# matthiasverstraete/3d_recognizer

Measured on AMD Instinct MI355X. Metric: training clouds/sec, N=40960 pts, bs=8, at 1/2/4/8 GPUs; mIoU parity, higher is better.
Workload: dtype f32 storage/accumulate, bf16x3 MFMA in the wide GEMMs

## Files before the change

### 3d_recognizer_amd/csrc/csr.hip

```cpp
#include "rl_common.h"

namespace {

constexpr int CSR_MAX_TASKS = 8;

struct CsrTask {
    const int32_t* idx;
    int n_src, k, n_dst;
    int32_t* offsets;
    int32_t* entries;
    int32_t* tmp;
    int32_t* cursor;
    int32_t* long_list;
    int32_t* long_count;
    int long_cap;
    int cap;
    int nbuckets;
    int ntiles;
    int32_t* bsize;
    int32_t* bstart;
};
struct CsrMulti {
    CsrTask t[CSR_MAX_TASKS];
    int ntasks;
    int B;
    int xcd;
};

__device__ __forceinline__ void csr_deal(const CsrMulti& m, int& b, int& bx) {
    if (m.xcd) {
        const int lin = (int)blockIdx.x + (int)gridDim.x * b;
        b = lin % m.B;
        bx = lin / m.B;
    }
}

__global__ __launch_bounds__(256) void csr_zero_kernel(const CsrMulti m) {
    const CsrTask& T = m.t[blockIdx.y];
    const long total = (long)m.B * T.n_dst;
    for (long e = (long)blockIdx.x * 256 + threadIdx.x; e < total; e += (long)gridDim.x * 256) T.cursor[e] = 0;
    if (blockIdx.x == 0 && threadIdx.x == 0) T.long_count[0] = 0;
}

__global__ __launch_bounds__(256) void csr_count_kernel(const CsrMulti m) {
    const CsrTask& T = m.t[blockIdx.y];
    const unsigned per = (unsigned)T.n_src * (unsigned)T.k;
    const long total = (long)m.B * per;
    for (long e = (long)blockIdx.x * 256 + threadIdx.x; e < total; e += (long)gridDim.x * 256) {
        const unsigned b = (unsigned)e / per;
        const int j = T.idx[e];
        if ((unsigned)j < (unsigned)T.n_dst) atomicAdd(&T.cursor[(long)b * T.n_dst + j], 1);
    }
}

__global__ __launch_bounds__(1024) void csr_scan_kernel(const CsrMulti m) {
    __shared__ int part[1024];
    const int task = blockIdx.x / m.B, b = blockIdx.x % m.B, t = threadIdx.x;
    const CsrTask& T = m.t[task];
    int* cu = T.cursor + (long)b * T.n_dst;
    int* off = T.offsets + (long)b * (T.n_dst + 1);
    const int chunk = (T.n_dst + 1023) / 1024;
    const int lo = min(T.n_dst, t * chunk), hi = min(T.n_dst, lo + chunk);
    int s = 0;
    for (int i = lo; i < hi; ++i) s += cu[i];
    part[t] = s;
    __syncthreads();
    for (int o = 1; o < 1024; o <<= 1) {
        const int v = (t >= o) ? part[t - o] : 0;
// ... 5 lines not shown
    for (int i = lo; i < hi; ++i) {
        const int c = cu[i];
        off[i] = run;
        cu[i] = run;
        run += c;
    }
    if (t == 1023) off[T.n_dst] = part[1023];
}

__global__ __launch_bounds__(256) void csr_fill_kernel(const CsrMulti m) {
    const CsrTask& T = m.t[blockIdx.y];
    const unsigned per = (unsigned)T.n_src * (unsigned)T.k;
    const long total = (long)m.B * per;
    for (long e = (long)blockIdx.x * 256 + threadIdx.x; e < total; e += (long)gridDim.x * 256) {
        const unsigned b = (unsigned)e / per;
        const int j = T.idx[e];
        if ((unsigned)j >= (unsigned)T.n_dst) continue;
        const int pos = atomicAdd(&T.cursor[(long)b * T.n_dst + j], 1);
        T.tmp[(long)b * per + pos] = (int)((unsigned)e - b * per);
    }
}

constexpr int CSR_TILE = 4096;
constexpr int CSR_BUCKET = 256;
constexpr int CSR_MAX_BUCKETS = 1024;

__global__ __launch_bounds__(256) void csr2_zero_kernel(const CsrMulti m) {
    const CsrTask& T = m.t[blockIdx.y];
    const long total = (long)m.B * T.nbuckets;
    for (long e = (long)blockIdx.x * 256 + threadIdx.x; e < total; e += (long)gridDim.x * 256) T.bsize[e] = 0;
    if (blockIdx.x == 0 && threadIdx.x == 0) T.long_count[0] = 0;
}

__global__ __launch_bounds__(256) void csr2_hist_kernel(const CsrMulti m) {
    __shared__ int hist[CSR_MAX_BUCKETS];
    const int task = blockIdx.y / m.B;
    int b = blockIdx.y % m.B, bx = blockIdx.x;
    csr_deal(m, b, bx);
    const CsrTask& T = m.t[task];
    if (bx >= T.ntiles) return;
    const int per = T.n_src * T.k;
    for (int i = threadIdx.x; i < T.nbuckets; i += 256) hist[i] = 0;
    __syncthreads();
    const int32_t* idx = T.idx + (long)b * per;
    const int e0 = bx * CSR_TILE;
#pragma unroll 4
    for (int i = 0; i < CSR_TILE / 256; ++i) {
        const int e = e0 + i * 256 + threadIdx.x;
        if (e < per) {
            const int j = idx[e];
            if ((unsigned)j < (unsigned)T.n_dst) atomicAdd(&hist[j >> 8], 1);
        }
    }
    __syncthreads();
    for (int i = threadIdx.x; i < T.nbuckets; i += 256)
        if (hist[i] > 0) atomicAdd(&T.bsize[(long)b * T.nbuckets + i], hist[i]);
}

__global__ __launch_bounds__(1024) void csr2_scan_kernel(const CsrMulti m) {
    __shared__ int part[1024];
    const int task = blockIdx.x / m.B, b = blockIdx.x % m.B, t = threadIdx.x;
    const CsrTask& T = m.t[task];
    int* bs = T.bsize + (long)b * T.nbuckets;
    const int v = t < T.nbuckets ? bs[t] : 0;
    part[t] = v;
    __syncthreads();
    for (int o = 1; o < 1024; o <<= 1) {
        const int u = (t >= o) ? part[t - o] : 0;
        __syncthreads();
        part[t] += u;
        __syncthreads();
    }
    int* st = T.bstart + (long)b * (T.nbuckets + 1);
    if (t < T.nbuckets) {
        st[t] = part[t] - v;
        bs[t] = 0;
    }
    if (t == T.nbuckets - 1) st[T.nbuckets] = part[t];
}

__global__ __launch_bounds__(256) void csr2_scatter_kernel(const CsrMulti m) {
    __shared__ int hist[CSR_MAX_BUCKETS];
    const int task = blockIdx.y / m.B;
    int b = blockIdx.y % m.B, bx = blockIdx.x;
    csr_deal(m, b, bx);
    const CsrTask& T = m.t[task];
    if (bx >= T.ntiles) return;
    const int per = T.n_src * T.k;
    for (int i = threadIdx.x; i < T.nbuckets; i += 256) hist[i] = 0;
    __syncthreads();
    const int32_t* idx = T.idx + (long)b * per;
    const int e0 = bx * CSR_TILE;
    int jv[CSR_TILE / 256], rk[CSR_TILE / 256];
#pragma unroll
    for (int i = 0; i < CSR_TILE / 256; ++i) {
        const int e = e0 + i * 256 + threadIdx.x;
        jv[i] = -1;
        if (e < per) {
            const int j = idx[e];
            if ((unsigned)j < (unsigned)T.n_dst) {
                jv[i] = j;
                rk[i] = atomicAdd(&hist[j >> 8], 1);
            }
        }
    }
    __syncthreads();
    for (int i = threadIdx.x; i < T.nbuckets; i += 256) {
        const int c = hist[i];
        hist[i] = c > 0 ? atomicAdd(&T.bsize[(long)b * T.nbuckets + i], c) : 0;
    }
    __syncthreads();
    const int* st = T.bstart + (long)b * (T.nbuckets + 1);
    int32_t* mid = T.tmp + (long)b * per;
#pragma unroll
    for (int i = 0; i < CSR_TILE / 256; ++i) {
        if (jv[i] >= 0) {
            const int h = jv[i] >> 8;
            mid[st[h] + hist[h] + rk[i]] = ((jv[i] & 255) << 24) | (e0 + i * 256 + threadIdx.x);
        }
    }
}

template <int CAP>
__global__ __launch_bounds__(256) void csr2_bucket_kernel(const CsrMulti m) {
    __shared__ int cnt[CSR_BUCKET], start[CSR_BUCKET], cur[CSR_BUCKET];
    __shared__ int seg[CSR_BUCKET][CAP + 1];
    const int task = blockIdx.y / m.B;
    int b = blockIdx.y % m.B, bx = blockIdx.x;
    csr_deal(m, b, bx);
    const CsrTask& T = m.t[task];
    if (T.cap != CAP || bx >= T.nbuckets) return;
    const int per = T.n_src * T.k, h = bx, t = threadIdx.x;
    const int* st = T.bstart + (long)b * (T.nbuckets + 1);
    const int s0 = st[h], mcount = st[h + 1] - s0;
    const int32_t* mid = T.tmp + (long)b * per + s0;
    int32_t* ent = T.entries + (long)b * per + s0;
    cnt[t] = 0;
    cur[t] = 0;
    __syncthreads();
    for (int e = t; e < mcount; e += 256) atomicAdd(&cnt[(unsigned)mid[e] >> 24], 1);
    __syncthreads();
    const int c = cnt[t];
    start[t] = c;
    __syncthreads();
    for (int o = 1; o < 256; o <<= 1) {
        const int u = (t >= o) ? start[t - o] : 0;
        __syncthreads();
        start[t] += u;
        __syncthreads();
    }
    const int my_start = start[t] - c;
    __syncthreads();
    start[t] = my_start;
    const int j = h * CSR_BUCKET + t;
    int* off = T.offsets + (long)b * (T.n_dst + 1);
    if (j < T.n_dst) off[j] = s0 + my_start;
    if (j == T.n_dst - 1) off[T.n_dst] = st[T.nbuckets];
    __syncthreads();
    for (int e = t; e < mcount; e += 256) {
        const int p = mid[e];
        const int lo = (unsigned)p >> 24, r = p & 0xffffff;
        const int pos = atomicAdd(&cur[lo], 1);
        if (cnt[lo] <= CAP) seg[lo][pos] = r;
        else ent[start[lo] + pos] = r;
// ... 230 lines not shown
    p.long_list = o;  o += up256((size_t)p.long_cap * 4);
    p.long_count = o; o += 256;
    p.bsize = o;      o += up256((size_t)B * p.nbuckets * 4);
    p.bstart = o;     o += up256((size_t)B * (p.nbuckets + 1) * 4);
    p.bytes = o;
    return p;
}
inline bool all_two_level(const rl_csr_task* tasks, int ntasks) {
    for (int i = 0; i < ntasks; ++i)
        if (!two_level_ok(tasks[i])) return false;
    return true;
}

}

extern "C" int64_t rl_csr_workspace_bytes(const rl_csr_task* tasks, int ntasks, int B) {
    if (!tasks || ntasks <= 0 || B <= 0) return 0;
    int64_t total = 0;
    for (int i = 0; i < ntasks; ++i) {
        if (tasks[i].n_src <= 0 || tasks[i].k <= 0 || tasks[i].n_dst <= 0) return 0;
        total += (int64_t)make_plan(B, tasks[i], all_two_level(tasks, ntasks)).bytes;
    }
    return total;
}

extern "C" int rl_csr_build(const rl_csr_task* tasks, int ntasks, int B, void* workspace, int64_t workspace_bytes,
                            void* stream) {
    RL_REQUIRE(tasks && ntasks > 0 && ntasks <= CSR_MAX_TASKS && B > 0 && (long)B * ntasks <= 65535, RL_ERR_ARGS,
               "rl_csr_build: 1..%d tasks expected", CSR_MAX_TASKS);
    RL_REQUIRE(workspace && ((uintptr_t)workspace & 255) == 0, RL_ERR_ARGS, "rl_csr_build: workspace must be 256-byte aligned");
    CsrMulti m;
    m.ntasks = ntasks;
    m.B = B;
    m.xcd = (B > 1 && 8 % B == 0) ? 1 : 0;
    char* ws = (char*)workspace;
    int64_t used = 0;
    long max_ent = 1, max_dst = 1;
    int max_tiles = 1, max_buckets = 1;
    bool need[3] = {false, false, false};
    for (int i = 0; i < ntasks; ++i)
        RL_REQUIRE(tasks[i].idx && tasks[i].offsets && tasks[i].entries && tasks[i].n_src > 0 && tasks[i].k > 0 && tasks[i].n_dst > 0,
                   RL_ERR_ARGS, "rl_csr_build: bad task %d", i);
    const bool two = all_two_level(tasks, ntasks);
    for (int i = 0; i < ntasks; ++i) {
        const rl_csr_task& t = tasks[i];
        RL_REQUIRE((int64_t)B * t.n_src * t.k < (1l << 31) && (int64_t)B * t.n_dst < (1l << 31), RL_ERR_ARGS,
                   "rl_csr_build: task %d is too large", i);
        const Plan p = make_plan(B, t, two);
        RL_REQUIRE(used + (int64_t)p.bytes <= workspace_bytes, RL_ERR_ARGS, "rl_csr_build: workspace too small");
        CsrTask& T = m.t[i];
        T.idx = t.idx; T.n_src = t.n_src; T.k = t.k; T.n_dst = t.n_dst; T.offsets = t.offsets; T.entries = t.entries;
        T.tmp = (int32_t*)(ws + used + p.tmp);
        T.cursor = (int32_t*)(ws + used + p.cursor);
        T.long_list = (int32_t*)(ws + used + p.long_list);
        T.long_count = (int32_t*)(ws + used + p.long_count);
        T.bsize = (int32_t*)(ws + used + p.bsize);
        T.bstart = (int32_t*)(ws + used + p.bstart);
        T.long_cap = p.long_cap; T.cap = p.cap; T.nbuckets = p.nbuckets; T.ntiles = p.ntiles;
        need[p.cap == 32 ? 0 : (p.cap == 64 || p.cap == 56) ? 1 : 2] = true;
        used += (int64_t)p.bytes;
        max_ent = max_ent > (long)B * t.n_src * t.k ? max_ent : (long)B * t.n_src * t.k;
        max_dst = max_dst > (long)B * t.n_dst ? max_dst : (long)B * t.n_dst;
        max_tiles = max_tiles > p.ntiles ? max_tiles : p.ntiles;
        max_buckets = max_buckets > p.nbuckets ? max_buckets : p.nbuckets;
    }
    hipStream_t st = (hipStream_t)stream;
    auto gridx = [](long work, int per) { long g = (work + per - 1) / per; return (unsigned)(g < 1 ? 1 : (g > 4096 ? 4096 : g)); };
    if (two) {
        hipLaunchKernelGGL(csr2_zero_kernel, dim3(gridx((long)B * max_buckets, 256), ntasks), dim3(256), 0, st, m);
        hipLaunchKernelGGL(csr2_hist_kernel, dim3(max_tiles, ntasks * B), dim3(256), 0, st, m);
        hipLaunchKernelGGL(csr2_scan_kernel, dim3(ntasks * B), dim3(1024), 0, st, m);
        hipLaunchKernelGGL(csr2_scatter_kernel, dim3(max_tiles, ntasks * B), dim3(256), 0, st, m);
        if (need[0]) hipLaunchKernelGGL(csr2_bucket_kernel<32>, dim3(max_buckets, ntasks * B), dim3(256), 0, st, m);
        if (need[1]) hipLaunchKernelGGL(csr2_bucket_kernel<56>, dim3(max_buckets, ntasks * B), dim3(256), 0, st, m);
        hipLaunchKernelGGL(csr2_sort_long_kernel, dim3(128, ntasks), dim3(256), 0, st, m);
        rl_note_kernel("csr2_bucket_kernel");
        RL_LAUNCH_CHECK("rl_csr_build");
        return RL_OK;
    }
    hipLaunchKernelGGL(csr_zero_kernel, dim3(gridx(max_dst, 256), ntasks), dim3(256), 0, st, m);
    hipLaunchKernelGGL(csr_count_kernel, dim3(gridx(max_ent, 256), ntasks), dim3(256), 0, st, m);
    hipLaunchKernelGGL(csr_scan_kernel, dim3(ntasks * B), dim3(1024), 0, st, m);
    hipLaunchKernelGGL(csr_fill_kernel, dim3(gridx(max_ent, 256), ntasks), dim3(256), 0, st, m);
    if (need[0]) hipLaunchKernelGGL((csr_sort_kernel<32, 256>), dim3(gridx(max_dst, 256), ntasks), dim3(256), 0, st, m);
    if (need[1]) hipLaunchKernelGGL((csr_sort_kernel<64, 128>), dim3(gridx(max_dst, 128), ntasks), dim3(128), 0, st, m);
    if (need[2]) hipLaunchKernelGGL((csr_sort_kernel<128, 64>), dim3(gridx(max_dst, 64), ntasks), dim3(64), 0, st, m);
    hipLaunchKernelGGL(csr_sort_long_kernel, dim3(128, ntasks), dim3(256), 0, st, m);
    rl_note_kernel("csr_sort_kernel");
    RL_LAUNCH_CHECK("rl_csr_build");
    return RL_OK;
}

extern "C" int rl_segment_sum_rows(const rl_segsum_desc* d, void* stream) {
    RL_REQUIRE(d && d->src && d->dst && d->offsets && d->entries && d->B > 0 && d->n_dst > 0 && d->C > 0 && d->entries_per_cloud >= 0,
               RL_ERR_ARGS, "rl_segment_sum_rows: bad descriptor");
    RL_REQUIRE(d->lds >= d->C && d->ldd >= d->C && d->dst_bstride >= d->n_dst && d->src_bstride > 0, RL_ERR_ARGS,
               "rl_segment_sum_rows: bad strides");
    RL_REQUIRE((int64_t)d->B * d->n_dst < (1l << 31), RL_ERR_ARGS, "rl_segment_sum_rows: too many rows");
    SegParams p;
    p.src = d->src; p.lds = d->lds; p.src_bstride = d->src_bstride; p.dst = d->dst; p.ldd = d->ldd;
    p.dst_bstride = d->dst_bstride; p.offsets = d->offsets; p.entries = d->entries; p.n_dst = d->n_dst; p.C = d->C;
    p.per = d->entries_per_cloud; p.total = (long)d->B * d->n_dst; p.accumulate = d->accumulate;
    p.xcd_chunk = 0;
    hipStream_t st = (hipStream_t)stream;
    const bool vec = (d->C % 4 == 0) && (d->lds % 4 == 0) && (d->ldd % 4 == 0) && ((uintptr_t)d->dst & 15) == 0 &&
                     ((uintptr_t)d->src & (d->src_bf16 ? 7 : 15)) == 0;
    RL_REQUIRE(!d->src_bf16 || vec, RL_ERR_UNSUPPORTED, "rl_segment_sum_rows: bf16 source rows need C, lds, ldd multiples of 4 and aligned tensors");
// ... 33 lines not shown
```

### 3d_recognizer_amd/csrc/knn_grid.hip

```cpp
#include "rl_common.h"
#include <stdlib.h>

namespace {

constexpr int KNN_SB = 3;


struct GridGeom {
    float lo[3];
    float inv[3];
    float h[3];
    int n[3];
    int ncell;
    float slack;
};

__device__ __forceinline__ unsigned enc(float f) {
    const unsigned u = __float_as_uint(f);
    return (u & 0x80000000u) ? ~u : (u | 0x80000000u);
}
__device__ __forceinline__ float dec(unsigned u) {
    return __uint_as_float((u & 0x80000000u) ? (u & 0x7fffffffu) : ~u);
}

constexpr int KNN_MAX_TASKS = 8;

struct KTask {
    const float* S;
    long s_bs;
    const float* Q;
    long q_bs;
    int Ns, Nq, k, self_mode;
    int32_t* idx32;
    int64_t* idx64;
    float* d2;
    GridGeom* geom;
    unsigned* bbox;
    int* count;
    int* start;
    int* cursor;
    float4* sorted;
    int cstride, maxcells;
    float per_cell;
    int lanes;
};

struct KMulti {
    int ntasks, B;
    int xcd;
    KTask t[KNN_MAX_TASKS];
};

__device__ __forceinline__ void knn_deal(const KMulti& m, int& b, int& bx) {
    if (m.xcd) {
        const int lin = (int)blockIdx.x + (int)gridDim.x * b;
        b = lin % m.B;
        bx = lin / m.B;
    }
}

__device__ __forceinline__ int kmax_of(int k) { return k == 1 ? 1 : k <= 4 ? 4 : k <= 8 ? 8 : k <= 16 ? 16 : k <= 32 ? 32 : 64; }

__global__ __launch_bounds__(256) void grid_init_kernel(const KMulti m) {
    const int task = blockIdx.y / m.B, b = blockIdx.y % m.B;
    const KTask& T = m.t[task];
    const int i = blockIdx.x * 256 + threadIdx.x;
    if (i < 6) T.bbox[b * 6 + i] = (i < 3) ? 0xffffffffu : 0u;
    int* cnt = T.count + (size_t)b * T.cstride;
    for (int e = i; e < T.cstride; e += gridDim.x * 256) cnt[e] = 0;
}

__global__ __launch_bounds__(256) void grid_bbox_kernel(const KMulti m) {
    const int task = blockIdx.y / m.B, b = blockIdx.y % m.B;
    const KTask& T = m.t[task];
    if (blockIdx.x * 256 >= T.Ns) return;
    const float* Sb = T.S + (size_t)b * T.s_bs * 3;
    float mn[3] = {INFINITY, INFINITY, INFINITY}, mx[3] = {-INFINITY, -INFINITY, -INFINITY};
    for (int j = blockIdx.x * 256 + threadIdx.x; j < T.Ns; j += gridDim.x * 256) {
#pragma unroll
        for (int a = 0; a < 3; ++a) {
            const float v = Sb[(size_t)j * 3 + a];
            mn[a] = fminf(mn[a], v);
            mx[a] = fmaxf(mx[a], v);
        }
    }
#pragma unroll
    for (int a = 0; a < 3; ++a) {
#pragma unroll
        for (int o = 32; o > 0; o >>= 1) {
            mn[a] = fminf(mn[a], __shfl_xor(mn[a], o, 64));
            mx[a] = fmaxf(mx[a], __shfl_xor(mx[a], o, 64));
        }
// ... 44 lines not shown
        g.n[a] = n;
        total *= n;
    }
    while (total > T.maxcells) {
        int a = 0;
        if (g.n[1] > g.n[a]) a = 1;
        if (g.n[2] > g.n[a]) a = 2;
        g.n[a] = (g.n[a] + 1) / 2;
        total = (long)g.n[0] * g.n[1] * g.n[2];
    }
    for (int a = 0; a < 3; ++a) {
        g.h[a] = (ext[a] > 0.f) ? ext[a] / (float)g.n[a] : 1.f;
        g.inv[a] = 1.f / g.h[a];
    }
    g.ncell = (int)total;
    g.slack = 1e-5f * extent + 1e-30f;
    T.geom[b] = g;
}

__device__ __forceinline__ void cell_coords(const GridGeom& g, float x, float y, float z, int c[3]) {
    const float p[3] = {x, y, z};
#pragma unroll
    for (int a = 0; a < 3; ++a) {
        int ci = (int)floorf((p[a] - g.lo[a]) * g.inv[a]);
        ci = ci < 0 ? 0 : ci;
        ci = ci >= g.n[a] ? g.n[a] - 1 : ci;
        c[a] = ci;
    }
}
__device__ __forceinline__ int cell_id(const GridGeom& g, const int c[3]) {
    return (c[2] * g.n[1] + c[1]) * g.n[0] + c[0];
}

__global__ __launch_bounds__(256) void grid_count_kernel(const KMulti m) {
    const int task = blockIdx.y / m.B, b = blockIdx.y % m.B;
    const KTask& T = m.t[task];
    const int j = blockIdx.x * 256 + threadIdx.x;
    if (j >= T.Ns) return;
    const GridGeom g = T.geom[b];
    const float* p = T.S + ((size_t)b * T.s_bs + j) * 3;
    int c[3];
    cell_coords(g, p[0], p[1], p[2], c);
    atomicAdd(&T.count[(size_t)b * T.cstride + cell_id(g, c)], 1);
}

__global__ __launch_bounds__(1024) void grid_scan_kernel(const KMulti m) {
    __shared__ int part[1024];
    const int task = blockIdx.x / m.B, b = blockIdx.x % m.B, t = threadIdx.x;
    const KTask& T = m.t[task];
    const int ncell = T.geom[b].ncell;
    const int* cnt = T.count + (size_t)b * T.cstride;
    int* st = T.start + (size_t)b * T.cstride;
    int* cu = T.cursor + (size_t)b * T.cstride;
    const int chunk = (ncell + 1023) / 1024;
    const int lo = t * chunk, hi = min(ncell, lo + chunk);
    int s = 0;
    for (int i = lo; i < hi; ++i) s += cnt[i];
    part[t] = s;
    __syncthreads();
    for (int o = 1; o < 1024; o <<= 1) {
        const int v = (t >= o) ? part[t - o] : 0;
        __syncthreads();
        part[t] += v;
        __syncthreads();
    }
    int run = part[t] - s;
    for (int i = lo; i < hi; ++i) {
        st[i] = run;
        cu[i] = run;
        run += cnt[i];
    }
    if (t == 1023) st[ncell] = part[1023];
}

__global__ __launch_bounds__(256) void grid_scatter_kernel(const KMulti m) {
    const int task = blockIdx.y / m.B, b = blockIdx.y % m.B;
    const KTask& T = m.t[task];
    const int j = blockIdx.x * 256 + threadIdx.x;
    if (j >= T.Ns) return;
    const GridGeom g = T.geom[b];
    const float* p = T.S + ((size_t)b * T.s_bs + j) * 3;
    int c[3];
    cell_coords(g, p[0], p[1], p[2], c);
    const int pos = atomicAdd(&T.cursor[(size_t)b * T.cstride + cell_id(g, c)], 1);
    T.sorted[(size_t)b * T.Ns + pos] = make_float4(p[0], p[1], p[2], __int_as_float(j));
}

constexpr unsigned long long KEY_EMPTY = 0x7FF0000000000000ull;
template <int KMAX>
__device__ __forceinline__ void insert_key(unsigned long long key, unsigned long long (&best)[KMAX]) {
    double kd = __builtin_bit_cast(double, key);
#pragma unroll
    for (int s = 0; s < KMAX; ++s) {
        const double bs = __builtin_bit_cast(double, best[s]);
        double lo, hi;
        asm("v_min_f64 %0, %1, %2" : "=v"(lo) : "v"(kd), "v"(bs));
        asm("v_max_f64 %0, %1, %2" : "=v"(hi) : "v"(kd), "v"(bs));
        best[s] = __builtin_bit_cast(unsigned long long, lo);
        kd = hi;
    }
}

template <int KMAX, int SB>
__device__ __forceinline__ void take_batch(const float4 (&cand)[SB], unsigned valid, float qx, float qy, float qz,
                                           unsigned long long (&best)[KMAX]) {
    unsigned long long key[SB];
    unsigned pass = 0;
#pragma unroll
    for (int i = 0; i < SB; ++i) {
        const float4 c = cand[i];
        const float dx = __fsub_rn(qx, c.x), dy = __fsub_rn(qy, c.y), dz = __fsub_rn(qz, c.z);
        const float d = __fadd_rn(__fadd_rn(__fmul_rn(dx, dx), __fmul_rn(dy, dy)), __fmul_rn(dz, dz));
        key[i] = ((unsigned long long)__float_as_uint(d) << 32) | (unsigned)__float_as_int(c.w);
        if (((valid >> i) & 1u) && key[i] < best[KMAX - 1]) pass |= 1u << i;
    }
    while (pass) {
        const int i = __ffs(pass) - 1;
        pass &= pass - 1;
        unsigned long long kk = key[0];
#pragma unroll
        for (int j = 1; j < SB; ++j)
            if (j == i) kk = key[j];
        insert_key<KMAX>(kk, best);
    }
}

template <int KMAX>
__device__ __forceinline__ void scan_range(const float4* __restrict__ pts, int begin, int end, float qx, float qy,
                                           float qz, unsigned long long (&best)[KMAX]) {
    constexpr int SB = KNN_SB;
    for (int t = begin; t < end; t += SB) {
        float4 cand[SB];
        unsigned valid = 0;
#pragma unroll
        for (int i = 0; i < SB; ++i) {
            cand[i] = pts[min(t + i, end - 1)];
            if (t + i < end) valid |= 1u << i;
        }
        take_batch<KMAX, SB>(cand, valid, qx, qy, qz, best);
    }
}

__device__ __forceinline__ int centre_out(int t) { return (t & 1) ? -((t + 1) >> 1) : (t >> 1); }

__device__ __forceinline__ float axis_gap(const GridGeom& g, int a, int ci, float q) {
    const float lo = g.lo[a] + (float)ci * g.h[a];
    const float hi = lo + g.h[a];
    float gap = fmaxf(lo - q, q - hi);
    gap -= g.slack;
    return gap > 0.f ? gap : 0.f;
}

template <int KMAX>
__device__ __forceinline__ void query_one_lane(const KTask& T, int b, int bx) {
    const int k = T.k, Nq = T.Nq, Ns = T.Ns;
    const int t = bx * 256 + threadIdx.x;
    if (t >= Nq) return;
    const int self_mode = T.self_mode;
    const float* Q = T.Q;
    const long q_bs = T.q_bs;
    int32_t* idx32 = T.idx32;
    int64_t* idx64 = T.idx64;
    float* d2out = T.d2;
    const GridGeom g = T.geom[b];
    const float4* pts = T.sorted + (size_t)b * Ns;
    const int* st = T.start + (size_t)b * T.cstride;
    float qx, qy, qz;
    int qi;
    if (self_mode) {
        const float4 me = pts[t];
        qx = me.x; qy = me.y; qz = me.z;
        qi = __float_as_int(me.w);
    } else {
        const float* p = Q + ((size_t)b * q_bs + t) * 3;
        qx = p[0]; qy = p[1]; qz = p[2];
        qi = t;
    }
    int c[3];
    cell_coords(g, qx, qy, qz, c);
    unsigned long long best[KMAX];
#pragma unroll
    for (int s = 0; s < KMAX; ++s) best[s] = KEY_EMPTY;

    const float q3[3] = {qx, qy, qz};
    for (int r = 0;; ++r) {
        const int z0 = max(c[2] - r, 0), z1 = min(c[2] + r, g.n[2] - 1);
        const int y0 = max(c[1] - r, 0), y1 = min(c[1] + r, g.n[1] - 1);
        const int x0 = max(c[0] - r, 0), x1 = min(c[0] + r, g.n[0] - 1);
        for (int tz = 0; tz <= 2 * r; ++tz) {
            const int z = c[2] + centre_out(tz);
            if (z < z0 || z > z1) continue;
            const bool zedge = (z == c[2] - r) || (z == c[2] + r);
            const float dz = axis_gap(g, 2, z, qz);
            for (int ty = 0; ty <= 2 * r; ++ty) {
                const int y = c[1] + centre_out(ty);
                if (y < y0 || y > y1) continue;
                const bool full_row = zedge || y == c[1] - r || y == c[1] + r;
                const float dy = axis_gap(g, 1, y, qy);
                const float dyz = dy * dy + dz * dz;
                const int row = (z * g.n[1] + y) * g.n[0];
                unsigned long long kth = best[KMAX - 1];
                if (k != KMAX) {
#pragma unroll
                    for (int s = 0; s < KMAX; ++s)
                        if (s == k - 1) kth = best[s];
                }
                const bool have = kth != KEY_EMPTY;
                const float lim = have ? __uint_as_float((unsigned)(kth >> 32)) * 1.00001f + 1e-30f : INFINITY;
                if (dyz > lim) continue;
                if (full_row) {
                    int xa = x0, xb = x1;
                    while (xa <= xb) {
                        const float gx = axis_gap(g, 0, xa, qx);
                        if (gx * gx + dyz > lim) ++xa; else break;
                    }
                    while (xb >= xa) {
                        const float gx = axis_gap(g, 0, xb, qx);
                        if (gx * gx + dyz > lim) --xb; else break;
                    }
                    if (xa <= xb) scan_range<KMAX>(pts, st[row + xa], st[row + xb + 1], qx, qy, qz, best);
                } else {
#pragma unroll
                    for (int e = 0; e < 2; ++e) {
                        const int x = e == 0 ? c[0] - r : c[0] + r;
                        if (x < x0 || x > x1 || (e == 1 && r == 0)) continue;
                        const float dxg = axis_gap(g, 0, x, qx);
                        if (dxg * dxg + dyz > lim) continue;
                        scan_range<KMAX>(pts, st[row + x], st[row + x + 1], qx, qy, qz, best);
                    }
                }
            }
        }
        const bool covers = (c[0] - r <= 0) && (c[0] + r >= g.n[0] - 1) && (c[1] - r <= 0) && (c[1] + r >= g.n[1] - 1) &&
                            (c[2] - r <= 0) && (c[2] + r >= g.n[2] - 1);
        if (covers) break;
        unsigned long long kth = best[KMAX - 1];
#pragma unroll
        for (int s = 0; s < KMAX; ++s)
            if (s == k - 1) kth = best[s];
        if (kth != KEY_EMPTY) {
            float bound = INFINITY;
#pragma unroll
            for (int a = 0; a < 3; ++a) {
                if (c[a] - r > 0) bound = fminf(bound, q3[a] - (g.lo[a] + (float)(c[a] - r) * g.h[a]));
                if (c[a] + r < g.n[a] - 1) bound = fminf(bound, (g.lo[a] + (float)(c[a] + r + 1) * g.h[a]) - q3[a]);
            }
            bound -= g.slack;
            const float kd = __uint_as_float((unsigned)(kth >> 32));
            if (bound > 0.f && kd < bound * bound * 0.999999f) break;
        }
    }
    const size_t o = ((size_t)b * Nq + qi) * k;
#pragma unroll
    for (int s = 0; s < KMAX; ++s) {
        if (s < k) {
            const bool empty = best[s] == KEY_EMPTY;
            const unsigned id = empty ? 0xffffffffu : (unsigned)(best[s] & 0xffffffffull);
            if (idx32) idx32[o + s] = (int32_t)id;
            if (idx64) idx64[o + s] = (int64_t)id;
            d2out[o + s] = __uint_as_float(empty ? 0xffffffffu : (unsigned)(best[s] >> 32));
        }
    }
}

template <int LANES>
__device__ __forceinline__ unsigned long long group_min(unsigned long long v) {
#pragma unroll
// ... 134 lines not shown
        }
    }
#pragma unroll
    for (int s = 0; s < KMAX; ++s) lists[qslot][sub][s] = best[s];
    __syncthreads();
    if (active) {
        const size_t o = ((size_t)b * Nq + qi) * k;
#pragma unroll
        for (int s = 0; s < KMAX; ++s) {
            const unsigned long long key = best[s];
            if (key == KEY_EMPTY) continue;
            int rank = s;
#pragma unroll
            for (int j = 1; j < LANES; ++j) {
                const unsigned long long* L = lists[qslot][(sub + j) % LANES];
                int lo = 0;
#pragma unroll
                for (int w = KMAX / 2; w >= 1; w >>= 1)
                    if (L[lo + w - 1] < key) lo += w;
                if (lo < KMAX && L[lo] < key) ++lo;
                rank += lo;
            }
            if (rank < k) {
                const unsigned id = (unsigned)(key & 0xffffffffull);
                if (T.idx32) T.idx32[o + rank] = (int32_t)id;
                if (T.idx64) T.idx64[o + rank] = (int64_t)id;
                T.d2[o + rank] = __uint_as_float((unsigned)(key >> 32));
            }
        }
    }
}

template <int KMAX>
__global__ __launch_bounds__(256, KMAX <= 16 ? 4 : 1) void grid_query_kernel(const KMulti m) {
    __shared__ unsigned long long lds[KMAX <= 16 ? 256 * KMAX : 1];
    const int task = blockIdx.y / m.B;
    int b = blockIdx.y % m.B, bx = blockIdx.x;
    knn_deal(m, b, bx);
    const KTask& T = m.t[task];
    if (kmax_of(T.k) != KMAX) return;
    if constexpr (KMAX <= 16) {
        if (T.lanes == 4) { query_n_lanes<KMAX, 4>(T, b, bx, lds); return; }
        if (T.lanes == 2) { query_n_lanes<KMAX, 2>(T, b, bx, lds); return; }
    }
    query_one_lane<KMAX>(T, b, bx);
}

struct Plan {
    int maxcells, cstride;
    float per_cell;
    size_t off_geom, off_bbox, off_count, off_start, off_cursor, off_sorted, bytes;
};

Plan make_plan(int B, int Ns, int k) {
    Plan p;
    constexpr float occ = 0.5f;
    p.per_cell = fmaxf(2.f, occ * (float)k);
    const long want = (long)((double)Ns / p.per_cell) + 1;
    p.maxcells = (int)(4 * want + 64);
    p.cstride = p.maxcells + 1;
    size_t o = 0;
    auto take = [&](size_t n) { size_t at = o; o += (n + 255) & ~(size_t)255; return at; };
    p.off_geom = take(sizeof(GridGeom) * B);
    p.off_bbox = take(sizeof(unsigned) * 6 * B);
    p.off_count = take(sizeof(int) * (size_t)p.cstride * B);
    p.off_start = take(sizeof(int) * (size_t)p.cstride * B);
    p.off_cursor = take(sizeof(int) * (size_t)p.cstride * B);
    p.off_sorted = take(sizeof(float4) * (size_t)Ns * B);
    p.bytes = o;
    return p;
}

void bind(KTask* t, const Plan& p, char* w) {
    t->geom = (GridGeom*)(w + p.off_geom);
    t->bbox = (unsigned*)(w + p.off_bbox);
    t->count = (int*)(w + p.off_count);
    t->start = (int*)(w + p.off_start);
    t->cursor = (int*)(w + p.off_cursor);
    t->sorted = (float4*)(w + p.off_sorted);
    t->cstride = p.cstride;
    t->maxcells = p.maxcells;
    t->per_cell = p.per_cell;
}

inline int lanes_for(long queries, int k) {
    if (k > 16) return 1;
    return queries >= 16384 ? 1 : 4;
}

int run_multi(const KMulti& m_in, hipStream_t st) {
    KMulti m = m_in;
    m.xcd = (m.B > 1 && 8 % m.B == 0) ? 1 : 0;
    for (int i = 0; i < m.ntasks; ++i) m.t[i].lanes = lanes_for((long)m.B * m.t[i].Nq, m.t[i].k);
    int maxNs = 1, maxNq = 1, maxc = 1;
    bool need[6] = {false, false, false, false, false, false};
    for (int i = 0; i < m.ntasks; ++i) {
        maxNs = max(maxNs, m.t[i].Ns);
        maxNq = max(maxNq, m.t[i].Nq);
        maxc = max(maxc, m.t[i].cstride);
        const int k = m.t[i].k;
        need[k == 1 ? 0 : k <= 4 ? 1 : k <= 8 ? 2 : k <= 16 ? 3 : k <= 32 ? 4 : 5] = true;
    }
    const int clouds = m.ntasks * m.B;
    int gi = rl_cdiv(maxc, 256);
    if (gi > 64) gi = 64;
    hipLaunchKernelGGL(grid_init_kernel, dim3(gi, clouds), dim3(256), 0, st, m);
    int gb = rl_cdiv(maxNs, 2048);
    if (gb > 16) gb = 16;
    hipLaunchKernelGGL(grid_bbox_kernel, dim3(gb, clouds), dim3(256), 0, st, m);
    hipLaunchKernelGGL(grid_geom_kernel, dim3(rl_cdiv(clouds, 64)), dim3(64), 0, st, m);
    hipLaunchKernelGGL(grid_count_kernel, dim3(rl_cdiv(maxNs, 256), clouds), dim3(256), 0, st, m);
    hipLaunchKernelGGL(grid_scan_kernel, dim3(clouds), dim3(1024), 0, st, m);
    hipLaunchKernelGGL(grid_scatter_kernel, dim3(rl_cdiv(maxNs, 256), clouds), dim3(256), 0, st, m);
    int gxq = 1;
    for (int i = 0; i < m.ntasks; ++i) gxq = max(gxq, rl_cdiv((long)m.t[i].Nq * m.t[i].lanes, 256));
    dim3 grid(gxq, clouds);
    if (need[0]) hipLaunchKernelGGL((grid_query_kernel<1>), grid, dim3(256), 0, st, m);
    if (need[1]) hipLaunchKernelGGL((grid_query_kernel<4>), grid, dim3(256), 0, st, m);
    if (need[2]) hipLaunchKernelGGL((grid_query_kernel<8>), grid, dim3(256), 0, st, m);
    if (need[3]) hipLaunchKernelGGL((grid_query_kernel<16>), grid, dim3(256), 0, st, m);
    if (need[4]) hipLaunchKernelGGL((grid_query_kernel<32>), grid, dim3(256), 0, st, m);
    if (need[5]) hipLaunchKernelGGL((grid_query_kernel<64>), grid, dim3(256), 0, st, m);
    rl_note_kernel("grid_query_kernel");
    RL_LAUNCH_CHECK("rl_knn(grid)");
    return RL_OK;
}

}

int64_t rl_knn_grid_workspace_bytes(int B, int Ns, int k) { return (int64_t)make_plan(B, Ns, k).bytes; }

int rl_knn_grid_run(const float* S, long s_bs, const float* Q, long q_bs, int B, int Ns, int Nq, int k, int32_t* i32,
                    int64_t* i64, float* d2, void* workspace, int64_t workspace_bytes, hipStream_t st) {
    const Plan p = make_plan(B, Ns, k);
    RL_REQUIRE(workspace && workspace_bytes >= (int64_t)p.bytes, RL_ERR_ARGS, "rl_knn: workspace too small (%ld < %ld bytes)",
               (long)workspace_bytes, (long)p.bytes);
    RL_REQUIRE(((uintptr_t)workspace & 255) == 0, RL_ERR_ARGS, "rl_knn: workspace must be 256-byte aligned");
    KMulti m;
    m.ntasks = 1;
    m.B = B;
    KTask& t = m.t[0];
    t.S = S; t.s_bs = s_bs; t.Q = Q; t.q_bs = q_bs; t.Ns = Ns; t.Nq = Nq; t.k = k;
    t.self_mode = (S == Q && s_bs == q_bs && Ns == Nq) ? 1 : 0;
    t.idx32 = i32; t.idx64 = i64; t.d2 = d2;
    bind(&t, p, (char*)workspace);
    return run_multi(m, st);
}

extern "C" int64_t rl_knn_multi_workspace_bytes(const rl_knn_task* tasks, int ntasks, int B) {
    if (!tasks || ntasks <= 0 || B <= 0) return 0;
    int64_t total = 0;
    for (int i = 0; i < ntasks; ++i) total += (int64_t)make_plan(B, tasks[i].Ns, tasks[i].k).bytes;
    return total;
}

// ... 28 lines not shown
```

### 3d_recognizer_amd/csrc/rl_common.h

```cpp
#pragma once
#include <hip/hip_runtime.h>
#include <stdarg.h>
#include <stdint.h>
#include <stdio.h>

#include "../../include/rl_randlanet.h"

void rl_set_error(const char* fmt, ...);
void rl_note_kernel(const char* name);

#define RL_REQUIRE(cond, code, ...)      \
    do {                                 \
        if (!(cond)) {                   \
            rl_set_error(__VA_ARGS__);   \
            return (code);               \
        }                                \
    } while (0)

#define RL_LAUNCH_CHECK(name)                                                        \
    do {                                                                             \
        hipError_t e_ = hipGetLastError();                                           \
        if (e_ != hipSuccess) {                                                      \
            rl_set_error("%s: launch failed: %s", name, hipGetErrorString(e_));      \
            return RL_ERR_LAUNCH;                                                    \
        }                                                                            \
    } while (0)

void rl_count_launch();
#undef hipLaunchKernelGGL
#define hipLaunchKernelGGL(kernelName, numBlocks, numThreads, memPerBlock, streamId, ...)                         \
    do {                                                                                                         \
        rl_count_launch();                                                                                       \
        kernelName<<<(numBlocks), (numThreads), (memPerBlock), (streamId)>>>(__VA_ARGS__);                       \
    } while (0)

int rl_wide_terms();

static inline int rl_cdiv(long a, long b) { return (int)((a + b - 1) / b); }

#include <stdlib.h>
static inline bool rl_float_atomics_allowed() {
    const char* e = getenv("RL_ALLOW_FLOAT_ATOMICS");
    return e && e[0] == '1';
}

static inline int rl_row_blocks_host(long rows, int rows_per_tile) {
    long tiles = (rows + rows_per_tile - 1) / rows_per_tile;
    if (tiles < 1) tiles = 1;
    return (int)(tiles < RL_MAX_SLOTS ? tiles : RL_MAX_SLOTS);
}

#define RL_ACT_NONE 0
#define RL_ACT_RELU 1
#define RL_ACT_LRELU 2

__device__ __forceinline__ float rl_act(float z, int act, float slope) {
    if (act == RL_ACT_RELU) return z > 0.f ? z : 0.f;
    if (act == RL_ACT_LRELU) return z > 0.f ? z : z * slope;
    return z;
}
__device__ __forceinline__ float rl_act_grad(float z, int act, float slope) {
    if (act == RL_ACT_RELU) return z > 0.f ? 1.f : 0.f;
    if (act == RL_ACT_LRELU) return z > 0.f ? 1.f : slope;
    return 1.f;
}

struct RlLazy {
    const float* scale;
    const float* shift;
    int act;
    float slope;
};
__device__ __forceinline__ float rl_lazy(const RlLazy& t, float raw, int c) {
    if (t.scale == nullptr) return raw;
    return rl_act(raw * t.scale[c] + t.shift[c], t.act, t.slope);
}

typedef __bf16 rl_bf16x4 __attribute__((ext_vector_type(4)));
template <bool BF>
__device__ __forceinline__ float rl_ldx(const float* p, long i) {
    if constexpr (BF) return (float)reinterpret_cast<const __bf16*>(p)[i];
    else return p[i];
// ... 60 lines not shown
```

Baseline: 1269.

## Pack multi-task launches into dense dealt grids and defer KNN k=16 inserts via LDS queue

Adds an RlDeal helper that turns per-task block counts into one dense 1D grid, sorted by size and optionally XCD-interleaved, so CSR and KNN kernels no longer launch max_tiles×tasks grids with idle early-exit blocks. The bucket kernels are launched only over tasks with a matching cap. For k=16, the one-lane KNN query now stages candidate keys in a per-thread LDS queue and merges them in wave-uniform batches, reducing divergent insertion-sort work. The two-lane query path is removed, and the queue adds LDS traffic and extra code paths.

Result: no change. 1276 (median of 6 runs) (+0.5%).

```diff
diff --git a/3d_recognizer_amd/csrc/csr.hip b/3d_recognizer_amd/csrc/csr.hip
--- a/3d_recognizer_amd/csrc/csr.hip
+++ b/3d_recognizer_amd/csrc/csr.hip
@@ -3,6 +3,7 @@
 namespace {
 
 constexpr int CSR_MAX_TASKS = 8;
+static_assert(CSR_MAX_TASKS <= RL_DEAL_MAX, "one RlDeal slot per task");
 
 struct CsrTask {
     const int32_t* idx;
@@ -24,16 +25,8 @@
     CsrTask t[CSR_MAX_TASKS];
     int ntasks;
     int B;
-    int xcd;
 };
 
-__device__ __forceinline__ void csr_deal(const CsrMulti& m, int& b, int& bx) {
-    if (m.xcd) {
-        const int lin = (int)blockIdx.x + (int)gridDim.x * b;
-        b = lin % m.B;
-        bx = lin / m.B;
-    }
-}
 
 __global__ __launch_bounds__(256) void csr_zero_kernel(const CsrMulti m) {
     const CsrTask& T = m.t[blockIdx.y];
@@ -105,13 +98,11 @@
     if (blockIdx.x == 0 && threadIdx.x == 0) T.long_count[0] = 0;
 }
 
-__global__ __launch_bounds__(256) void csr2_hist_kernel(const CsrMulti m) {
+__global__ __launch_bounds__(256) void csr2_hist_kernel(const CsrMulti m, const RlDeal deal) {
     __shared__ int hist[CSR_MAX_BUCKETS];
-    const int task = blockIdx.y / m.B;
-    int b = blockIdx.y % m.B, bx = blockIdx.x;
-    csr_deal(m, b, bx);
+    int task, b, bx;
+    if (!rl_deal_find(deal, task, b, bx)) return;
     const CsrTask& T = m.t[task];
-    if (bx >= T.ntiles) return;
     const int per = T.n_src * T.k;
     for (int i = threadIdx.x; i < T.nbuckets; i += 256) hist[i] = 0;
     __syncthreads();
@@ -152,13 +143,11 @@
     if (t == T.nbuckets - 1) st[T.nbuckets] = part[t];
 }
 
-__global__ __launch_bounds__(256) void csr2_scatter_kernel(const CsrMulti m) {
+__global__ __launch_bounds__(256) void csr2_scatter_kernel(const CsrMulti m, const RlDeal deal) {
     __shared__ int hist[CSR_MAX_BUCKETS];
-    const int task = blockIdx.y / m.B;
-    int b = blockIdx.y % m.B, bx = blockIdx.x;
-    csr_deal(m, b, bx);
+    int task, b, bx;
+    if (!rl_deal_find(deal, task, b, bx)) return;
     const CsrTask& T = m.t[task];
-    if (bx >= T.ntiles) return;
     const int per = T.n_src * T.k;
     for (int i = threadIdx.x; i < T.nbuckets; i += 256) hist[i] = 0;
     __syncthreads();
@@ -195,14 +184,13 @@
 }
 
 template <int CAP>
-__global__ __launch_bounds__(256) void csr2_bucket_kernel(const CsrMulti m) {
+__global__ __launch_bounds__(256) void csr2_bucket_kernel(const CsrMulti m, const RlDeal deal) {
     __shared__ int cnt[CSR_BUCKET], start[CSR_BUCKET], cur[CSR_BUCKET];
     __shared__ int seg[CSR_BUCKET][CAP + 1];
-    const int task = blockIdx.y / m.B;
-    int b = blockIdx.y % m.B, bx = blockIdx.x;
-    csr_deal(m, b, bx);
+    int task, b, bx;
+    if (!rl_deal_find(deal, task, b, bx)) return;
     const CsrTask& T = m.t[task];
-    if (T.cap != CAP || bx >= T.nbuckets) return;
+    if (bx >= T.nbuckets) return;
     const int per = T.n_src * T.k, h = bx, t = threadIdx.x;
     const int* st = T.bstart + (long)b * (T.nbuckets + 1);
     const int s0 = st[h], mcount = st[h + 1] - s0;
@@ -499,11 +487,12 @@
     CsrMulti m;
     m.ntasks = ntasks;
     m.B = B;
-    m.xcd = (B > 1 && 8 % B == 0) ? 1 : 0;
+    const bool xcd = B > 1 && 8 % B == 0;
     char* ws = (char*)workspace;
     int64_t used = 0;
     long max_ent = 1, max_dst = 1;
-    int max_tiles = 1, max_buckets = 1;
+    int max_buckets = 1;
+    int tiles[CSR_MAX_TASKS], buckets[2][CSR_MAX_TASKS];
     bool need[3] = {false, false, false};
     for (int i = 0; i < ntasks; ++i)
         RL_REQUIRE(tasks[i].idx && tasks[i].offsets && tasks[i].entries && tasks[i].n_src > 0 && tasks[i].k > 0 && tasks[i].n_dst > 0,
@@ -528,18 +517,26 @@
         used += (int64_t)p.bytes;
         max_ent = max_ent > (long)B * t.n_src * t.k ? max_ent : (long)B * t.n_src * t.k;
         max_dst = max_dst > (long)B * t.n_dst ? max_dst : (long)B * t.n_dst;
-        max_tiles = max_tiles > p.ntiles ? max_tiles : p.ntiles;
+        tiles[i] = p.ntiles;
+        buckets[0][i] = p.cap == 32 ? 1 : 0;
+        buckets[1][i] = p.cap == 32 ? 0 : 1;
         max_buckets = max_buckets > p.nbuckets ? max_buckets : p.nbuckets;
     }
     hipStream_t st = (hipStream_t)stream;
     auto gridx = [](long work, int per) { long g = (work + per - 1) / per; return (unsigned)(g < 1 ? 1 : (g > 4096 ? 4096 : g)); };
     if (two) {
         hipLaunchKernelGGL(csr2_zero_kernel, dim3(gridx((long)B * max_buckets, 256), ntasks), dim3(256), 0, st, m);
-        hipLaunchKernelGGL(csr2_hist_kernel, dim3(max_tiles, ntasks * B), dim3(256), 0, st, m);
+        const RlDeal dt = rl_deal_make(tiles, ntasks, B, xcd);
+        for (int i = 0; i < ntasks; ++i) {
+            buckets[0][i] *= max_buckets;
+            buckets[1][i] *= max_buckets;
+        }
+        const RlDeal db32 = rl_deal_make(buckets[0], ntasks, B, xcd), db56 = rl_deal_make(buckets[1], ntasks, B, xcd);
+        hipLaunchKernelGGL(csr2_hist_kernel, rl_deal_grid(dt), dim3(256), 0, st, m, dt);
         hipLaunchKernelGGL(csr2_scan_kernel, dim3(ntasks * B), dim3(1024), 0, st, m);
-        hipLaunchKernelGGL(csr2_scatter_kernel, dim3(max_tiles, ntasks * B), dim3(256), 0, st, m);
-        if (need[0]) hipLaunchKernelGGL(csr2_bucket_kernel<32>, dim3(max_buckets, ntasks * B), dim3(256), 0, st, m);
-        if (need[1]) hipLaunchKernelGGL(csr2_bucket_kernel<56>, dim3(max_buckets, ntasks * B), dim3(256), 0, st, m);
+        hipLaunchKernelGGL(csr2_scatter_kernel, rl_deal_grid(dt), dim3(256), 0, st, m, dt);
+        if (need[0]) hipLaunchKernelGGL(csr2_bucket_kernel<32>, rl_deal_grid(db32), dim3(256), 0, st, m, db32);
+        if (need[1]) hipLaunchKernelGGL(csr2_bucket_kernel<56>, rl_deal_grid(db56), dim3(256), 0, st, m, db56);
         hipLaunchKernelGGL(csr2_sort_long_kernel, dim3(128, ntasks), dim3(256), 0, st, m);
         rl_note_kernel("csr2_bucket_kernel");
         RL_LAUNCH_CHECK("rl_csr_build");
diff --git a/3d_recognizer_amd/csrc/knn_grid.hip b/3d_recognizer_amd/csrc/knn_grid.hip
--- a/3d_recognizer_amd/csrc/knn_grid.hip
+++ b/3d_recognizer_amd/csrc/knn_grid.hip
@@ -24,6 +24,7 @@
 }
 
 constexpr int KNN_MAX_TASKS = 8;
+static_assert(KNN_MAX_TASKS <= RL_DEAL_MAX, "one RlDeal slot per task");
 
 struct KTask {
     const float* S;
@@ -47,17 +48,8 @@
 
 struct KMulti {
     int ntasks, B;
-    int xcd;
     KTask t[KNN_MAX_TASKS];
 };
-
-__device__ __forceinline__ void knn_deal(const KMulti& m, int& b, int& bx) {
-    if (m.xcd) {
-        const int lin = (int)blockIdx.x + (int)gridDim.x * b;
-        b = lin % m.B;
-        bx = lin / m.B;
-    }
-}
 
 __device__ __forceinline__ int kmax_of(int k) { return k == 1 ? 1 : k <= 4 ? 4 : k <= 8 ? 8 : k <= 16 ? 16 : k <= 32 ? 32 : 64; }
 
@@ -168,10 +160,11 @@
     return (c[2] * g.n[1] + c[1]) * g.n[0] + c[0];
 }
 
-__global__ __launch_bounds__(256) void grid_count_kernel(const KMulti m) {
-    const int task = blockIdx.y / m.B, b = blockIdx.y % m.B;
+__global__ __launch_bounds__(256) void grid_count_kernel(const KMulti m, const RlDeal deal) {
+    int task, b, bx;
+    if (!rl_deal_find(deal, task, b, bx)) return;
     const KTask& T = m.t[task];
-    const int j = blockIdx.x * 256 + threadIdx.x;
+    const int j = bx * 256 + threadIdx.x;
     if (j >= T.Ns) return;
     const GridGeom g = T.geom[b];
     const float* p = T.S + ((size_t)b * T.s_bs + j) * 3;
@@ -209,10 +202,11 @@
     if (t == 1023) st[ncell] = part[1023];
 }
 
-__global__ __launch_bounds__(256) void grid_scatter_kernel(const KMulti m) {
-    const int task = blockIdx.y / m.B, b = blockIdx.y % m.B;
+__global__ __launch_bounds__(256) void grid_scatter_kernel(const KMulti m, const RlDeal deal) {
+    int task, b, bx;
+    if (!rl_deal_find(deal, task, b, bx)) return;
     const KTask& T = m.t[task];
-    const int j = blockIdx.x * 256 + threadIdx.x;
+    const int j = bx * 256 + threadIdx.x;
     if (j >= T.Ns) return;
     const GridGeom g = T.geom[b];
     const float* p = T.S + ((size_t)b * T.s_bs + j) * 3;
@@ -261,9 +255,38 @@
     }
 }
 
+constexpr int KNN_QD = 8;
+template <int KMAX>
+constexpr bool knn_deferred = KMAX == 16;
+
+template <int KMAX>
+__device__ __forceinline__ void drain_queue(unsigned long long* q, int& n, unsigned long long (&best)[KMAX]) {
+    for (int j = 0; j < KNN_QD; ++j) {
+        if (!__any(n > 0)) break;
+        unsigned long long key = KEY_EMPTY;
+        if (n > 0) key = q[--n * 256];
+        insert_key<KMAX>(key, best);
+    }
+}
+
+template <int KMAX, int SB>
+__device__ __forceinline__ void queue_batch(const float4 (&cand)[SB], unsigned valid, float qx, float qy, float qz,
+                                            unsigned long long* q, int& n, unsigned long long (&best)[KMAX]) {
+    static_assert(SB < KNN_QD, "a queue takes at least one batch");
+#pragma unroll
+    for (int i = 0; i < SB; ++i) {
+        const float4 c = cand[i];
+        const float dx = __fsub_rn(qx, c.x), dy = __fsub_rn(qy, c.y), dz = __fsub_rn(qz, c.z);
+        const float d = __fadd_rn(__fadd_rn(__fmul_rn(dx, dx), __fmul_rn(dy, dy)), __fmul_rn(dz, dz));
+        const unsigned long long key = ((unsigned long long)__float_as_uint(d) << 32) | (unsigned)__float_as_int(c.w);
+        if (((valid >> i) & 1u) && key < best[KMAX - 1]) q[n++ * 256] = key;
+    }
+    if (__any(n > KNN_QD - SB)) drain_queue<KMAX>(q, n, best);
+}
+
 template <int KMAX>
 __device__ __forceinline__ void scan_range(const float4* __restrict__ pts, int begin, int end, float qx, float qy,
-                                           float qz, unsigned long long (&best)[KMAX]) {
+                                           float qz, unsigned long long* q, int& n, unsigned long long (&best)[KMAX]) {
     constexpr int SB = KNN_SB;
     for (int t = begin; t < end; t += SB) {
         float4 cand[SB];
@@ -273,7 +296,8 @@
             cand[i] = pts[min(t + i, end - 1)];
             if (t + i < end) valid |= 1u << i;
         }
-        take_batch<KMAX, SB>(cand, valid, qx, qy, qz, best);
+        if constexpr (knn_deferred<KMAX>) queue_batch<KMAX, SB>(cand, valid, qx, qy, qz, q, n, best);
+        else take_batch<KMAX, SB>(cand, valid, qx, qy, qz, best);
     }
 }
 
@@ -288,7 +312,7 @@
 }
 
 template <int KMAX>
-__device__ __forceinline__ void query_one_lane(const KTask& T, int b, int bx) {
+__device__ __forceinline__ void query_one_lane(const KTask& T, int b, int bx, unsigned long long* lds) {
     const int k = T.k, Nq = T.Nq, Ns = T.Ns;
     const int t = bx * 256 + threadIdx.x;
     if (t >= Nq) return;
@@ -317,6 +341,8 @@
     unsigned long long best[KMAX];
 #pragma unroll
     for (int s = 0; s < KMAX; ++s) best[s] = KEY_EMPTY;
+    unsigned long long* queue = lds + threadIdx.x;
+    int nq = 0;
 
     const float q3[3] = {qx, qy, qz};
     for (int r = 0;; ++r) {
@@ -354,7 +380,7 @@
                         const float gx = axis_gap(g, 0, xb, qx);
                         if (gx * gx + dyz > lim) --xb; else break;
                     }
-                    if (xa <= xb) scan_range<KMAX>(pts, st[row + xa], st[row + xb + 1], qx, qy, qz, best);
+                    if (xa <= xb) scan_range<KMAX>(pts, st[row + xa], st[row + xb + 1], qx, qy, qz, queue, nq, best);
                 } else {
 #pragma unroll
                     for (int e = 0; e < 2; ++e) {
@@ -362,13 +388,14 @@
                         if (x < x0 || x > x1 || (e == 1 && r == 0)) continue;
                         const float dxg = axis_gap(g, 0, x, qx);
                         if (dxg * dxg + dyz > lim) continue;
-                        scan_range<KMAX>(pts, st[row + x], st[row + x + 1], qx, qy, qz, best);
+                        scan_range<KMAX>(pts, st[row + x], st[row + x + 1], qx, qy, qz, queue, nq, best);
                     }
                 }
             }
         }
         const bool covers = (c[0] - r <= 0) && (c[0] + r >= g.n[0] - 1) && (c[1] - r <= 0) && (c[1] + r >= g.n[1] - 1) &&
                             (c[2] - r <= 0) && (c[2] + r >= g.n[2] - 1);
+        if constexpr (knn_deferred<KMAX>) drain_queue<KMAX>(queue, nq, best);
         if (covers) break;
         unsigned long long kth = best[KMAX - 1];
 #pragma unroll
@@ -569,18 +596,17 @@
 }
 
 template <int KMAX>
-__global__ __launch_bounds__(256, KMAX <= 16 ? 4 : 1) void grid_query_kernel(const KMulti m) {
+__global__ __launch_bounds__(256, KMAX <= 16 ? 4 : 1) void grid_query_kernel(const KMulti m, const RlDeal deal) {
     __shared__ unsigned long long lds[KMAX <= 16 ? 256 * KMAX : 1];
-    const int task = blockIdx.y / m.B;
-    int b = blockIdx.y % m.B, bx = blockIdx.x;
-    knn_deal(m, b, bx);
+    static_assert(!knn_deferred<KMAX> || KNN_QD <= KMAX, "the one-lane queues share the merge lists' LDS");
+    int task, b, bx;
+    if (!rl_deal_find(deal, task, b, bx)) return;
     const KTask& T = m.t[task];
     if (kmax_of(T.k) != KMAX) return;
     if constexpr (KMAX <= 16) {
         if (T.lanes == 4) { query_n_lanes<KMAX, 4>(T, b, bx, lds); return; }
-        if (T.lanes == 2) { query_n_lanes<KMAX, 2>(T, b, bx, lds); return; }
-    }
-    query_one_lane<KMAX>(T, b, bx);
+    }
+    query_one_lane<KMAX>(T, b, bx, lds);
 }
 
 struct Plan {
@@ -627,16 +653,25 @@
 
 int run_multi(const KMulti& m_in, hipStream_t st) {
     KMulti m = m_in;
-    m.xcd = (m.B > 1 && 8 % m.B == 0) ? 1 : 0;
-    for (int i = 0; i < m.ntasks; ++i) m.t[i].lanes = lanes_for((long)m.B * m.t[i].Nq, m.t[i].k);
-    int maxNs = 1, maxNq = 1, maxc = 1;
-    bool need[6] = {false, false, false, false, false, false};
+    const bool xcd = m.B > 1 && 8 % m.B == 0;
+    int maxNs = 1, maxc = 1;
+    constexpr int NBUCKET = 6;
+    int bs[KNN_MAX_TASKS], bq[NBUCKET][KNN_MAX_TASKS];
     for (int i = 0; i < m.ntasks; ++i) {
-        maxNs = max(maxNs, m.t[i].Ns);
-        maxNq = max(maxNq, m.t[i].Nq);
-        maxc = max(maxc, m.t[i].cstride);
-        const int k = m.t[i].k;
-        need[k == 1 ? 0 : k <= 4 ? 1 : k <= 8 ? 2 : k <= 16 ? 3 : k <= 32 ? 4 : 5] = true;
+        KTask& t = m.t[i];
+        t.lanes = lanes_for((long)m.B * t.Nq, t.k);
+        maxNs = max(maxNs, t.Ns);
+        maxc = max(maxc, t.cstride);
+        bs[i] = rl_cdiv(t.Ns, 256);
+        const int bucket = t.k == 1 ? 0 : t.k <= 4 ? 1 : t.k <= 8 ? 2 : t.k <= 16 ? 3 : t.k <= 32 ? 4 : 5;
+        for (int u = 0; u < NBUCKET; ++u) bq[u][i] = u == bucket ? rl_cdiv((long)t.Nq * t.lanes, 256) : 0;
+    }
+    const RlDeal ds = rl_deal_make(bs, m.ntasks, m.B, false);
+    RL_REQUIRE(rl_deal_total(ds) >= 0, RL_ERR_ARGS, "rl_knn: too many workgroups for one launch");
+    RlDeal dq[NBUCKET];
+    for (int u = 0; u < NBUCKET; ++u) {
+        dq[u] = rl_deal_make(bq[u], m.ntasks, m.B, xcd);
+        RL_REQUIRE(rl_deal_total(dq[u]) >= 0, RL_ERR_ARGS, "rl_knn: too many workgroups for one launch");
     }
     const int clouds = m.ntasks * m.B;
     int gi = rl_cdiv(maxc, 256);
@@ -646,18 +681,15 @@
     if (gb > 16) gb = 16;
     hipLaunchKernelGGL(grid_bbox_kernel, dim3(gb, clouds), dim3(256), 0, st, m);
     hipLaunchKernelGGL(grid_geom_kernel, dim3(rl_cdiv(clouds, 64)), dim3(64), 0, st, m);
-    hipLaunchKernelGGL(grid_count_kernel, dim3(rl_cdiv(maxNs, 256), clouds), dim3(256), 0, st, m);
+    hipLaunchKernelGGL(grid_count_kernel, rl_deal_grid(ds), dim3(256), 0, st, m, ds);
     hipLaunchKernelGGL(grid_scan_kernel, dim3(clouds), dim3(1024), 0, st, m);
-    hipLaunchKernelGGL(grid_scatter_kernel, dim3(rl_cdiv(maxNs, 256), clouds), dim3(256), 0, st, m);
-    int gxq = 1;
-    for (int i = 0; i < m.ntasks; ++i) gxq = max(gxq, rl_cdiv((long)m.t[i].Nq * m.t[i].lanes, 256));
-    dim3 grid(gxq, clouds);
-    if (need[0]) hipLaunchKernelGGL((grid_query_kernel<1>), grid, dim3(256), 0, st, m);
-    if (need[1]) hipLaunchKernelGGL((grid_query_kernel<4>), grid, dim3(256), 0, st, m);
-    if (need[2]) hipLaunchKernelGGL((grid_query_kernel<8>), grid, dim3(256), 0, st, m);
-    if (need[3]) hipLaunchKernelGGL((grid_query_kernel<16>), grid, dim3(256), 0, st, m);
-    if (need[4]) hipLaunchKernelGGL((grid_query_kernel<32>), grid, dim3(256), 0, st, m);
-    if (need[5]) hipLaunchKernelGGL((grid_query_kernel<64>), grid, dim3(256), 0, st, m);
+    hipLaunchKernelGGL(grid_scatter_kernel, rl_deal_grid(ds), dim3(256), 0, st, m, ds);
+    if (dq[0].count) hipLaunchKernelGGL((grid_query_kernel<1>), rl_deal_grid(dq[0]), dim3(256), 0, st, m, dq[0]);
+    if (dq[1].count) hipLaunchKernelGGL((grid_query_kernel<4>), rl_deal_grid(dq[1]), dim3(256), 0, st, m, dq[1]);
+    if (dq[2].count) hipLaunchKernelGGL((grid_query_kernel<8>), rl_deal_grid(dq[2]), dim3(256), 0, st, m, dq[2]);
+    if (dq[3].count) hipLaunchKernelGGL((grid_query_kernel<16>), rl_deal_grid(dq[3]), dim3(256), 0, st, m, dq[3]);
+    if (dq[4].count) hipLaunchKernelGGL((grid_query_kernel<32>), rl_deal_grid(dq[4]), dim3(256), 0, st, m, dq[4]);
+    if (dq[5].count) hipLaunchKernelGGL((grid_query_kernel<64>), rl_deal_grid(dq[5]), dim3(256), 0, st, m, dq[5]);
     rl_note_kernel("grid_query_kernel");
     RL_LAUNCH_CHECK("rl_knn(grid)");
     return RL_OK;
diff --git a/3d_recognizer_amd/csrc/rl_common.h b/3d_recognizer_amd/csrc/rl_common.h
--- a/3d_recognizer_amd/csrc/rl_common.h
+++ b/3d_recognizer_amd/csrc/rl_common.h
@@ -48,6 +48,66 @@
     long tiles = (rows + rows_per_tile - 1) / rows_per_tile;
     if (tiles < 1) tiles = 1;
     return (int)(tiles < RL_MAX_SLOTS ? tiles : RL_MAX_SLOTS);
+}
+
+constexpr int RL_DEAL_MAX = 8;
+constexpr int RL_DEAL_GX = 1 << 20;
+struct RlDeal {
+    int count, B, xcd;
+    int first[RL_DEAL_MAX + 1];
+    int nblk[RL_DEAL_MAX];
+    int task[RL_DEAL_MAX];
+};
+static inline RlDeal rl_deal_make(const int* blocks, int ntasks, int B, bool xcd) {
+    RlDeal d;
+    d.count = 0;
+    d.B = B;
+    d.xcd = xcd ? 1 : 0;
+    for (int s = 0; s < RL_DEAL_MAX; ++s) d.nblk[s] = d.task[s] = 0;
+    for (int i = 0; i < ntasks && i < RL_DEAL_MAX; ++i) {
+        if (blocks[i] <= 0) continue;
+        int s = d.count++;
+        for (; s > 0 && d.nblk[s - 1] < blocks[i]; --s) {
+            d.nblk[s] = d.nblk[s - 1];
+            d.task[s] = d.task[s - 1];
+        }
+        d.nblk[s] = blocks[i];
+        d.task[s] = i;
+    }
+    long at = 0;
+    for (int s = 0; s < d.count; ++s) {
+        d.first[s] = (int)at;
+        at += (long)d.nblk[s] * B;
+    }
+    for (int s = d.count; s <= RL_DEAL_MAX; ++s) d.first[s] = at < 0x7fffffffl ? (int)at : -1;
+    return d;
+}
+static inline long rl_deal_total(const RlDeal& d) { return d.first[RL_DEAL_MAX]; }
+static inline dim3 rl_deal_grid(const RlDeal& d) {
+    const long total = rl_deal_total(d);
+    return total <= RL_DEAL_GX ? dim3((unsigned)total) : dim3(RL_DEAL_GX, (unsigned)((total + RL_DEAL_GX - 1) / RL_DEAL_GX));
+}
+__device__ __forceinline__ bool rl_deal_find(const RlDeal& d, int& task, int& b, int& bx) {
+    const int lin = (int)blockIdx.x + (int)gridDim.x * (int)blockIdx.y;
+    if (lin >= d.first[RL_DEAL_MAX]) return false;
+    int base = 0, n = d.nblk[0];
+    task = d.task[0];
+#pragma unroll
+    for (int i = 1; i < RL_DEAL_MAX; ++i) {
+        const bool in = lin >= d.first[i];
+        base = in ? d.first[i] : base;
+        n = in ? d.nblk[i] : n;
+        task = in ? d.task[i] : task;
+    }
+    const int local = lin - base;
+    if (d.xcd) {
+        b = local % d.B;
+        bx = local / d.B;
+    } else {
+        b = local / n;
+        bx = local % n;
+    }
+    return true;
 }
 
 #define RL_ACT_NONE 0
```
